# PN-CourseWork/02689-AdvancedNumericalAlgorithmP3

Hardware: AMD Instinct MI355X
Metric: steady-state time-steps/sec at N=256 Re=1000 (higher is better)
Workload: dtype f64; 1 GPU; solver=spectral (SG) N=256 Re=1000 fp64, full solve() iteration (dt, 4 RK stages + BCs, change/residual norms, E/Z/P), fluid from rest; N=256, trials_per_gpu=1, parallelism=1 independent trial(s), one per GPU

## Files before the change

02689-advancednumericalalgorithmp3_amd/csrc/ldc_kernels.hip:

```cpp

#include <hip/hip_runtime.h>
#include <stdint.h>
#include <stdlib.h>
#include <string.h>
#include <mutex>
#include <new>
#include <type_traits>
#include <vector>

#include "ldc_hip.h"
#include "ldc_fv_common.inc"

namespace {

#ifdef LDC_TIMING
#define LDC_ABL(x, bits) ((x).ablate & (bits))
#else
#define LDC_ABL(x, bits) 0
#endif

constexpr int kWaves = 4;
constexpr int kThreads = 256;
constexpr int kMfmaBounds = 512;

__device__ __forceinline__ v4d ldfrag(const double* X, int ld, int r0, int k0, int lane) {
  return *reinterpret_cast<const v4d*>(X + (size_t)(r0 + (lane & 15)) * ld + k0 + 4 * (lane >> 4));
}

#define LDC_GLOBAL __attribute__((address_space(1)))
__device__ __forceinline__ v4d ldpk(const double* XK, int NB, int R, int G, int lane) {
  return *(const LDC_GLOBAL v4d*)(XK + (((size_t)(R * NB + G) << 6) + lane) * 4);
}
template <typename T>
__device__ __forceinline__ T gl(const T* p, size_t i) {
  return ((const LDC_GLOBAL T*)p)[i];
}

__device__ __forceinline__ __amdgpu_buffer_rsrc_t raw_rsrc(const double* base) {
  return __builtin_amdgcn_make_buffer_rsrc((void*)base, 0, -1, 0x00020000);
}
typedef unsigned int v4u __attribute__((ext_vector_type(4)));
typedef double v2d_t __attribute__((ext_vector_type(2)));
template <bool COH>
__device__ __forceinline__ v4d ldpk_t(const double* XK, int NB, int R, int G, int lane) {
  if constexpr (!COH) {
    return ldpk(XK, NB, R, G, lane);
  } else {
    const __amdgpu_buffer_rsrc_t r = raw_rsrc(XK);
    const int off = ((((R * NB + G) << 6) + lane) * 4) * (int)sizeof(double);
    const v2d_t lo = __builtin_bit_cast(v2d_t, __builtin_amdgcn_raw_buffer_load_b128(r, off, 0, 16));
    const v2d_t hi = __builtin_bit_cast(v2d_t, __builtin_amdgcn_raw_buffer_load_b128(r, off + 16, 0, 16));
    return (v4d){lo[0], lo[1], hi[0], hi[1]};
  }
}
template <bool COH, typename T>
__device__ __forceinline__ T gl_t(const T* p, size_t i) {
  if constexpr (!COH) return gl(p, i);
  else return __hip_atomic_load((const LDC_GLOBAL T*)p + i, __ATOMIC_RELAXED, __HIP_MEMORY_SCOPE_AGENT);
}

__device__ __forceinline__ void st_out2(double* p, double v0, double v1, int wt) {
  const v2d_t v = {v0, v1};
  if (wt) asm volatile("global_store_dwordx4 %0, %1, off sc1\n\ts_nop 1" :: "v"((LDC_GLOBAL v2d_t*)p), "v"(v) : "memory");
  else *(LDC_GLOBAL v2d_t*)p = v;
}
__device__ __forceinline__ void st_out(double* p, double v, int wt) {
  if (wt) __hip_atomic_store((LDC_GLOBAL double*)p, v, __ATOMIC_RELAXED, __HIP_MEMORY_SCOPE_AGENT);
  else *(LDC_GLOBAL double*)p = v;
}

template <typename T>
__device__ __forceinline__ T sload(const T* p) {
  return *(const __attribute__((address_space(4))) T*)p;
}

template <int CTRL>
__device__ __forceinline__ double dpp_move(double x) {
  const long long b = __builtin_bit_cast(long long, x);
  const int lo = __builtin_amdgcn_update_dpp(0, (int)b, CTRL, 0xf, 0xf, true);
  const int hi = __builtin_amdgcn_update_dpp(0, (int)(b >> 32), CTRL, 0xf, 0xf, true);
  return __builtin_bit_cast(double, ((long long)hi << 32) | (unsigned int)lo);
}
__device__ __forceinline__ double lane_value(double x, int l) {
  const long long b = __builtin_bit_cast(long long, x);
  const int lo = __builtin_amdgcn_readlane((int)b, l), hi = __builtin_amdgcn_readlane((int)(b >> 32), l);
  return __builtin_bit_cast(double, ((long long)hi << 32) | (unsigned int)lo);
// ... 2521 lines not shown
```

02689-advancednumericalalgorithmp3_amd/csrc/ldc_wide_kernel.inc:

```

constexpr int kWT = 16;
constexpr int kWTmin = 6;
constexpr int kWD2 = 6;
constexpr int kWD = 4;

struct WArgs {
  int M, LD, NB, T;
  int tail;
  int Mx, My;
  int with_diag;
  double nu, beta2;
  const double *DxK, *D2xK, *DyK, *D2yK, *GxFK, *GyFK;
  const double *ulid, *wx, *wy;
  double *U, *UT, *V, *VT, *P;
  double *UK[3], *UTK[3], *VK[3], *VTK[3], *PK[3];
  double *PTK[3];
  double *WK, *WTK;
  const double *IxF, *IyF;
  const double *Dx, *D2x, *Dy, *D2y, *GxF, *GyF;
  const double *DxL, *D2xL, *DyL, *D2yL;
  double* wedge;
  double* jobs;
  double* ring;
  double* rvec;
  double *part4, *partZ0, *partP0;
  long long stride;
  FinalArgs fin;
  unsigned* flags;
  unsigned* giveup;
  double* stamps;
};
constexpr int kWStampPoints = 12;
constexpr int kWStampsPerWg = kStageWaves * 4 * kWStampPoints;

struct WLaunch {
  int B, n_iters;
  const WArgs* trials;
  WArgs one;
};
static_assert(sizeof(WLaunch) <= 4096, "WLaunch must fit the kernel-argument segment");
typedef const __attribute__((address_space(4))) WArgs WArgsC;

struct WLds {
  int OPS, RES, AXY, RNG, EYX, RY, TOT, RSUM, TOTAL;
};
__host__ __device__ inline WLds wlds_of(int T) {
  WLds l;
  l.OPS = 0;
  l.RES = l.OPS + 4 * T * 256;
// ... 55 lines not shown
  }
}
__device__ __forceinline__ void wgive_up(WArgsC& a, TrialState* S) {
  S->abort = 1;
  __hip_atomic_store((LDC_GLOBAL unsigned*)a.giveup, 1u, __ATOMIC_RELAXED, __HIP_MEMORY_SCOPE_AGENT);
}

__device__ __forceinline__ bool wbar(WArgsC& a, unsigned& phaseA, int T, int bx, int I, int J, int tid, TrialState* S, bool all,
                                     double* stp = nullptr) {
  asm volatile("s_waitcnt vmcnt(0)" ::: "memory");
  WSTAMP(7);
  __syncthreads();
  WSTAMP(8);
  ++phaseA;
  if (tid < 64) {
    if (tid == 0) __hip_atomic_store((LDC_GLOBAL unsigned*)a.flags + 32 * bx, phaseA, __ATOMIC_RELAXED, __HIP_MEMORY_SCOPE_AGENT);
    if (!wwait_flags(a.flags, phaseA, T, I, J, all, tid) && tid == 0) wgive_up(a, S);
    WSTAMP(9);
  }
  __syncthreads();
  WSTAMP(10);
  return S->abort == 0;
}

__device__ __forceinline__ v4d wld4(const double* base, size_t i) {
  const __amdgpu_buffer_rsrc_t r = raw_rsrc(base);
  const int off = (int)(i * sizeof(double));
  const v2d_t lo = __builtin_bit_cast(v2d_t, __builtin_amdgcn_raw_buffer_load_b128(r, off, 0, 16));
  const v2d_t hi = __builtin_bit_cast(v2d_t, __builtin_amdgcn_raw_buffer_load_b128(r, off + 16, 0, 16));
  return (v4d){lo[0], lo[1], hi[0], hi[1]};
}
__device__ __forceinline__ int wrows_padded(int nwg) { return (nwg + 3) & ~3; }

template <bool CONST_A>
__device__ __forceinline__ void wchain2(v4d& r0, v4d& r1, const double* p0, const double* p1, const double* pan, int NB,
                                        int prow, int T, int lane) {
  constexpr int D = kWD2;
  v4d f[D];
#pragma unroll
  for (int d = 0; d < D; ++d) {
    f[d] = ldpk_t<true>(pan, NB, prow, d, lane);
    __builtin_amdgcn_sched_barrier(0);
  }
  v4d c0[2], c1[2];
#pragma unroll
  for (int h = 0; h < 2; ++h) { c0[h] = (v4d){0.0, 0.0, 0.0, 0.0}; c1[h] = (v4d){0.0, 0.0, 0.0, 0.0}; }
  auto mm = [&](const v4d& x, int g) {
    const v4d k0 = wfrag_lds(p0 + g * 256, lane), k1 = wfrag_lds(p1 + g * 256, lane);
#pragma unroll
    for (int s = 0; s < 4; ++s) {
      if (CONST_A) { c0[s & 1] = MFMA_F64(k0[s], x[s], c0[s & 1]); c1[s & 1] = MFMA_F64(k1[s], x[s], c1[s & 1]); }
      else         { c0[s & 1] = MFMA_F64(x[s], k0[s], c0[s & 1]); c1[s & 1] = MFMA_F64(x[s], k1[s], c1[s & 1]); }
    }
  };
  int g = 0;
  for (; g + 2 * D <= T; g += D) {
#pragma unroll
    for (int d = 0; d < D; ++d) {
      mm(f[d], g + d);
      f[d] = ldpk_t<true>(pan, NB, prow, g + d + D, lane);
      __builtin_amdgcn_sched_barrier(0);
    }
  }
  const int rest = T - g - D;
#pragma unroll
  for (int d = 0; d < D; ++d) {
    mm(f[d], g + d);
    if (d < rest) f[d] = ldpk_t<true>(pan, NB, prow, g + d + D, lane);
  }
#pragma unroll
  for (int d = 0; d < D; ++d)
    if (d < rest) mm(f[d], g + D + d);
  r0 = xadd(c0[0], c0[1]);
  r1 = xadd(c1[0], c1[1]);
}

template <bool OP_LDS, bool CONST_A>
__device__ __forceinline__ v4d wchain1(const double* opl, const double* opk, int oprow, const double* pan, int prow, int NB,
                                       int ng, int lane, int g0 = 0) {
  constexpr int D = kWD;
  v4d f[D], o[D];
#pragma unroll
  for (int d = 0; d < D; ++d) {
    f[d] = ldpk_t<true>(pan, NB, prow, g0 + (d < ng ? d : ng - 1), lane);
    if (!OP_LDS) o[d] = ldpk(opk, NB, oprow, g0 + (d < ng ? d : ng - 1), lane);
    __builtin_amdgcn_sched_barrier(0);
  }
  v4d c[4];
#pragma unroll
  for (int s = 0; s < 4; ++s) c[s] = (v4d){0.0, 0.0, 0.0, 0.0};
  auto mm = [&](const v4d& x, const v4d& k) {
#pragma unroll
    for (int s = 0; s < 4; ++s) c[s] = CONST_A ? MFMA_F64(k[s], x[s], c[s]) : MFMA_F64(x[s], k[s], c[s]);
  };
  int g = 0;
  for (; g + 2 * D <= ng; g += D) {
#pragma unroll
    for (int d = 0; d < D; ++d) {
      mm(f[d], OP_LDS ? wfrag_lds(opl + (g0 + g + d) * 256, lane) : o[d]);
      f[d] = ldpk_t<true>(pan, NB, prow, g0 + g + d + D, lane);
      if (!OP_LDS) o[d] = ldpk(opk, NB, oprow, g0 + g + d + D, lane);
      __builtin_amdgcn_sched_barrier(0);
    }
  }
  const int rest = ng - g - D;
#pragma unroll
  for (int d = 0; d < D; ++d) {
    if (g + d < ng) mm(f[d], OP_LDS ? wfrag_lds(opl + (g0 + g + d) * 256, lane) : o[d]);
    if (d < rest) {
      f[d] = ldpk_t<true>(pan, NB, prow, g0 + g + d + D, lane);
      if (!OP_LDS) o[d] = ldpk(opk, NB, oprow, g0 + g + d + D, lane);
    }
  }
#pragma unroll
  for (int d = 0; d < D; ++d)
    if (d < rest) mm(f[d], OP_LDS ? wfrag_lds(opl + (g0 + g + D + d) * 256, lane) : o[d]);
  return xadd(xadd(c[0], c[1]), xadd(c[2], c[3]));
}

__device__ __forceinline__ void wput(double* lds, const WLds& Ld, int slot, const v4d& acc, int lane) {
#pragma unroll
  for (int r = 0; r < 4; ++r) lds[Ld.RES + (slot * 4 + r) * 64 + lane] = acc[r];
}

__device__ __forceinline__ double wave_total(double x) { return quad_sum(row16_sum(x)); }
__device__ __forceinline__ double wave_top(double x) { return quad_max(row16_max(x)); }


__device__ __forceinline__ void wring_partials(WArgsC& a, const WLds& Ld, const XNode& n, double* lds, double pn, int bx,
                                               int lane, int wv) {
  double* dst = a.ring + (size_t)wopaque_s(bx) * 64;
  const double eyc[2] = {lds[Ld.EYX + n.tj], lds[Ld.EYX + 16 + n.tj]};
  const double exc[2] = {lds[Ld.EYX + 32 + n.ti], lds[Ld.EYX + 48 + n.ti]};
#pragma unroll
  for (int c = 0; c < 2; ++c) {
    const double r = row16_sum(pn * eyc[c]);
    if ((lane & 15) == 0) wst1(dst + c * 16 + n.ti, r);
    const double q = quad_sum(exc[c] * pn);
    if (lane < 16) lds[Ld.RY + (wv * 2 + c) * 16 + lane] = q;
  }
}
__device__ __forceinline__ void wring_partials_finish(WArgsC& a, const WLds& Ld, const double* lds, int bx, int tid) {
  if (tid < 32) {
    const double* r = lds + Ld.RY + tid;
// ... 12 lines not shown
  double s = 0.0;
#pragma unroll
  for (int L = 0; L < kWT; ++L) s += (L < T) ? t[L] : 0.0;
  wst1(a.rvec + (size_t)v * 16 * T + 16 * B + r, s);
}
__device__ __forceinline__ void wvec_line(const double* vec, size_t off, const double* opK, int oprow, int NB, int T, int lane_,
                                          double* out, const double* opl = nullptr) {
  const int lane = wopaque(lane_);
  double s = 0.0;
#pragma unroll
  for (int g0 = 0; g0 < kWT; g0 += 8) {
    if (g0 < T) {
      v4d G[8], A[8];
#pragma unroll
      for (int g = 0; g < 8; ++g) {
        const int gc = g0 + g < T ? g0 + g : T - 1;
        if (opl == nullptr) G[g] = ldpk(opK, NB, oprow, gc, lane);
        A[g] = wld4(vec, off + 16 * gc + 4 * (lane >> 4));
      }
#pragma unroll
      for (int g = 0; g < 8; ++g) {
        if (g0 + g < T) {
          const v4d Gg = (opl == nullptr) ? G[g] : wfrag_lds(opl + (g0 + g) * 256, lane);
          s = nm_madd(Gg[0], A[g][0], s); s = nm_madd(Gg[1], A[g][1], s);
          s = nm_madd(Gg[2], A[g][2], s); s = nm_madd(Gg[3], A[g][3], s);
        }
      }
    }
  }
  s = quad_sum(s);
  if (lane < 16) out[lane] = s;
}
struct WVecHalf { double a[8]; };
__device__ __forceinline__ void wvec_issue(WVecHalf& h, const double* vec, size_t off, int g0, int ng, int lane_) {
  const int lane = wopaque(lane_);
#pragma unroll
  for (int g = 0; g < 8; ++g) h.a[g] = xld(vec, off + 16 * (g0 + (g < ng ? g : ng - 1)) + 4 * (lane >> 4) + (lane & 3));
}
__device__ __forceinline__ void wvec_finish(const WVecHalf& h, const double* opl, const double* opK, int oprow, int NB, int g0, int ng,
                                            int lane_, double* out) {
  const int lane = wopaque(lane_);
  v4d G[8];
  if (opl == nullptr) {
#pragma unroll
    for (int g = 0; g < 8; ++g) G[g] = ldpk(opK, NB, oprow, g0 + (g < ng ? g : ng - 1), lane);
  }
  double s0 = 0.0, s1 = 0.0, s2 = 0.0, s3 = 0.0;
#pragma unroll
  for (int g = 0; g < 8; ++g) {
    if (g < ng) {
      const v4d Gg = (opl == nullptr) ? G[g] : wfrag_lds(opl + (g0 + g) * 256, lane);
      s0 = nm_madd(Gg[0], dpp_move<0x00>(h.a[g]), s0); s1 = nm_madd(Gg[1], dpp_move<0x55>(h.a[g]), s1);
      s2 = nm_madd(Gg[2], dpp_move<0xAA>(h.a[g]), s2); s3 = nm_madd(Gg[3], dpp_move<0xFF>(h.a[g]), s3);
    }
  }
  const double s = quad_sum((s0 + s1) + (s2 + s3));
  if (lane < 16) out[lane] = s;
}
__device__ __forceinline__ void wring_line(WArgsC& a, int T, int blk, int lane, int kind, int c, double* out) {
  wvec_line(a.rvec, (size_t)(2 * kind + c) * 16 * T, kind == 0 ? a.GxFK : a.GyFK, blk, a.NB, T, lane, out);
}
__device__ __forceinline__ double wvv(const double* row, const double* vec, size_t off, int n, int lane_) {
  const int lane = wopaque(lane_);
  double s = 0.0;
  if (4 * lane < n) {
    const v4d r = *(const LDC_GLOBAL v4d*)(row + 4 * lane);
    const v4d x = wld4(vec, off + 4 * lane);
    s = nm_madd(r[0], x[0], s); s = nm_madd(r[1], x[1], s); s = nm_madd(r[2], x[2], s); s = nm_madd(r[3], x[3], s);
  }
  return wave_total(s);
// ... 28 lines not shown
  jb.cd[2] = xld(base, WJ_CD2 * 16 + r); jb.cd[3] = xld(base, WJ_CD3 * 16 + r);
  jb.ce[0] = xld(base, WJ_CE0 * 16 + r); jb.ce[1] = xld(base, WJ_CE1 * 16 + r);
  jb.ce[2] = xld(base, WJ_CE2 * 16 + r); jb.ce[3] = xld(base, WJ_CE3 * 16 + r);
  jb.pgs = xld(base, WJ_PGS * 16 + r); jb.pgr = xld(base, WJ_PGR * 16 + r);
  jb.omega = xld(base, WJ_OMEGA * 16 + r); jb.wq = xld(base, WJ_WQ * 16 + r); jb.opl = xld(base, WJ_OPL * 16 + r);
  jb.am1 = xld(base, WJ_UNI * 16 + 0); jb.am2 = xld(base, WJ_UNI * 16 + 1); jb.wc = xld(base, WJ_UNI * 16 + 2);
}
__device__ __forceinline__ void wjob_store(WArgsC& a, const WJob& jb, int T, int lane_, bool all) {
  const int lane = wopaque(lane_);
  double* base = a.jobs + (size_t)wjob_id(jb.kind, jb.blk, T) * kWJobDoubles;
  if (lane < 16) {
    wst1(base + WJ_PGS * 16 + lane, jb.pgs); wst1(base + WJ_PGR * 16 + lane, jb.pgr); wst1(base + WJ_OMEGA * 16 + lane, jb.omega);
    if (all) {
      wst1(base + WJ_UE * 16 + lane, jb.ue); wst1(base + WJ_VE * 16 + lane, jb.ve);
      wst1(base + WJ_CD0 * 16 + lane, jb.cd[0]); wst1(base + WJ_CD1 * 16 + lane, jb.cd[1]);
      wst1(base + WJ_CD2 * 16 + lane, jb.cd[2]); wst1(base + WJ_CD3 * 16 + lane, jb.cd[3]);
      wst1(base + WJ_CE0 * 16 + lane, jb.ce[0]); wst1(base + WJ_CE1 * 16 + lane, jb.ce[1]);
      wst1(base + WJ_CE2 * 16 + lane, jb.ce[2]); wst1(base + WJ_CE3 * 16 + lane, jb.ce[3]);
      wst1(base + WJ_WQ * 16 + lane, jb.wq); wst1(base + WJ_OPL * 16 + lane, jb.opl);
      if (lane == 0) { wst1(base + WJ_UNI * 16 + 0, jb.am1); wst1(base + WJ_UNI * 16 + 1, jb.am2); wst1(base + WJ_UNI * 16 + 2, jb.wc); }
    }
  }
}
enum { WR_JOBLINE = 64, WR_EXTRA = 96, WR_CGX = 97, WR_CGY = 98, WR_CPX = 99, WR_CPY = 100, WR_JOBRING2 = 104 };

struct WEdgeLoads { double ra[4], rb[4]; v4d f0[4], f1[4]; };
template <int MODE, bool DIAGV>
__device__ __forceinline__ void wedge_issue(WEdgeLoads& w, WArgsC& a, int kind, int blk, const XStageIo io, int T, int w4, int lane_) {
  const int lane = wopaque(lane_);
  const int NB = a.NB;
  const size_t rowm = (size_t)(a.M - 1) * a.LD;
  const double *pan0, *pan1, *rA, *rB;
  if (MODE == 1) {
    pan0 = kind == 0 ? a.VTK[io.in] : a.UK[io.in]; pan1 = kind == 0 ? a.PTK[io.pin] : a.PK[io.pin];
    rA = (kind == 0 ? a.Dx : a.Dy) + rowm; rB = (kind == 0 ? a.GxF : a.GyF) + rowm;
  } else if (MODE == 3) {
    pan0 = kind == 0 ? a.WTK : a.WK; pan1 = pan0;
    rA = (kind == 0 ? a.Dx : a.Dy) + rowm; rB = rA;
  } else {
    pan0 = kind == 0 ? a.UTK[io.in] : a.UK[io.in]; pan1 = kind == 0 ? a.VTK[io.in] : a.VK[io.in];
    rA = (kind == 0 ? a.Dx : a.Dy) + rowm; rB = (kind == 0 ? a.D2x : a.D2y) + rowm;
  }
  constexpr bool use0 = !(MODE == 1 && !DIAGV), use1 = MODE != 3;
#pragma unroll
  for (int m = 0; m < 4; ++m) {
    const int g = w4 + 4 * m, gc = g < T ? g : T - 1;
    const int ko = 16 * gc + 4 * (lane >> 4) + (lane & 3);
    w.ra[m] = *(const LDC_GLOBAL double*)(rA + ko);
    w.rb[m] = use1 ? *(const LDC_GLOBAL double*)(rB + ko) : w.ra[m];
    if (g >= T) { w.ra[m] = 0.0; w.rb[m] = 0.0; }
  }
#pragma unroll
  for (int m = 0; m < 4; ++m) {
    const int g = w4 + 4 * m, gc = g < T ? g : T - 1;
    w.f0[m] = use0 ? ldpk_t<true>(pan0, NB, blk, gc, lane) : (v4d){0.0, 0.0, 0.0, 0.0};
    w.f1[m] = use1 ? ldpk_t<true>(pan1, NB, blk, gc, lane) : w.f0[m];
  }
}
template <int MODE, bool DIAGV>
__device__ __forceinline__ void wedge_dots(const WEdgeLoads& w, const WLds& Ld, double* lds, int w4, int lane_) {
  const int lane = wopaque(lane_);
  constexpr bool use0 = !(MODE == 1 && !DIAGV), use1 = MODE != 3;
  double acc[4] = {0.0, 0.0, 0.0, 0.0};
#pragma unroll
  for (int m = 0; m < 4; ++m) {
    const v4d va = {dpp_move<0x00>(w.ra[m]), dpp_move<0x55>(w.ra[m]), dpp_move<0xAA>(w.ra[m]), dpp_move<0xFF>(w.ra[m])};
    v4d vb = va;
    if (use1) vb = (v4d){dpp_move<0x00>(w.rb[m]), dpp_move<0x55>(w.rb[m]), dpp_move<0xAA>(w.rb[m]), dpp_move<0xFF>(w.rb[m])};
    if (MODE == 1) { if (use0) fma4(acc[0], w.f0[m], va); fma4(acc[1], w.f1[m], vb); }
    if (MODE == 3) fma4(acc[0], w.f0[m], va);
    if (MODE == 4) {
#pragma unroll
      for (int e = 0; e < 4; ++e) {
        acc[0] = fma(w.f0[m][e], va[e], acc[0]); acc[1] = fma(w.f0[m][e], vb[e], acc[1]);
        acc[2] = fma(w.f1[m][e], va[e], acc[2]); acc[3] = fma(w.f1[m][e], vb[e], acc[3]);
      }
    }
  }
#pragma unroll
  for (int d = 0; d < 4; ++d) {
    if ((MODE == 1 && d < 2) || (MODE == 3 && d < 1) || MODE == 4) {
      const double x = quad_sum(acc[d]);
      if (lane < 16) lds[Ld.AXY + (w4 * 5 + (MODE == 3 ? 4 : d)) * 16 + lane] = x;
    }
  }
}
template <int MODE, bool DIAGV>
__device__ __forceinline__ void wedge_stream(WArgsC& a, const WLds& Ld, double* lds, int kind, int blk, const XStageIo io,
                                             int T, int w4, int lane) {
// ... 244 lines not shown
  constexpr bool PUBZ = DIAGV && K == 2;
  constexpr double alphas[4] = {0.25, 1.0 / 3.0, 0.5, 1.0};
  constexpr int bin[4] = {0, 1, 2, 1}, bout[4] = {1, 2, 1, 0};
  const XStageIo io = {bin[K], bout[K], bin[K], bout[K], alphas[K], K};
  const int T = wopaque_s(T_), bx = wopaque_s(bx_), I = wopaque_s(I_), J = wopaque_s(J_);
  WJob jb;
  jb.kind = TAIL ? jkind : -1; jb.blk = jblk;
  jb.ue = jb.ve = jb.am1 = jb.am2 = jb.pgs = jb.pgr = jb.omega = jb.wq = jb.opl = jb.wc = 0.0;
#pragma unroll
  for (int d = 0; d < 4; ++d) { jb.cd[d] = 0.0; jb.ce[d] = 0.0; }
  const int tid = wopaque((int)threadIdx.x), lane = tid & 63;
  const int wv = __builtin_amdgcn_readfirstlane(tid >> 6);
#ifdef LDC_TIMING
  double* const stp = stamp ? a.stamps + (size_t)bx * kWStampsPerWg + (wv * 4 + K) * kWStampPoints : nullptr;
#else
  double* const stp = nullptr; (void)stamp;
#endif
  WSTAMP(0);
  const int NB = a.NB, nwg = T * T;
  constexpr bool has_p = SP || LAST;
  const double* ops = lds + Ld.OPS;
  const int iLast = (a.Mx - 1) / 16, jLast = (a.My - 1) / 16;
  double* rsum = lds + Ld.RSUM;
  double* rng = lds + Ld.RNG;
  const bool job = TAIL && jb.kind >= 0;
  v4d fx[PS_N + 2];
  WFoldState fs = {false, false, 0.0, 0.0};
  WEdgeLoads jw;
  WVecHalf jvh;
  double wre = 0.0, wce = 0.0;
  if (wv < 4) {
    if (TAIL && DIAGE == 2) { wre = xld(a.wedge, (size_t)n.j); wce = xld(a.wedge, (size_t)16 * kWT + n.i); }
    const bool xrole = wv < 2;
    const double* pan = wv == 0 ? a.UTK[io.in] : wv == 1 ? a.VTK[io.in] : wv == 2 ? a.UK[io.in] : a.VK[io.in];
    const double* p0 = ops + (xrole ? 0 : 2) * T * 256;
    v4d c0, c1;
    if (xrole) wchain2<true>(c0, c1, p0, p0 + T * 256, pan, NB, J, T, lane);
    else wchain2<false>(c0, c1, p0, p0 + T * 256, pan, NB, I, T, lane);
    WSTAMP(1);
    wput(lds, Ld, wv == 0 ? XR_UX : wv == 1 ? XR_VX : wv == 2 ? XR_UY : XR_VY, c0, lane);
    wput(lds, Ld, wv == 0 ? XR_UXX : wv == 1 ? XR_VXX : wv == 2 ? XR_UYY : XR_VYY, c1, lane);
  } else {
    if (PUBZ && wv == 7 && lane == 0) {
      const double* r = rsum;
      const double x = (((r[0] + r[1]) + (r[2] + r[3])) + ((r[4] + r[5]) + (r[6] + r[7]))) +
                       (((r[8] + r[9]) + (r[10] + r[11])) + ((r[12] + r[13]) + (r[14] + r[15])));
      const int step0 = S->step;
      wst1(a.partZ0 + (size_t)((step0 > 0 ? step0 - 1 : 0) & 1) * a.stride + wopaque_s(bx), TAIL ? x + r[16] : x);
    }
    if (GPV) {
      constexpr bool THREE = !(SP && K == 3);
      const int c1 = THREE ? (2 * T + 1) / 3 : T;
      if (wv == 4) wput(lds, Ld, XR_PX, wchain1<false, true>(nullptr, a.GxFK, I, a.PTK[io.pin], J, NB, c1, lane), lane);
      else if (wv == 5) wput(lds, Ld, XR_PY, wchain1<false, false>(nullptr, a.GyFK, J, a.PK[io.pin], I, NB, c1, lane), lane);
      else if (THREE && wv == 6) {
        wput(lds, Ld, XR_WX, wchain1<false, true>(nullptr, a.GxFK, I, a.PTK[io.pin], J, NB, T - c1, lane, c1), lane);
        wput(lds, Ld, XR_WY, wchain1<false, false>(nullptr, a.GyFK, J, a.PK[io.pin], I, NB, T - c1, lane, c1), lane);
      }
    }
    if (AGRADW) {
      const int h0 = (T + 1) / 2, g0 = wv < 6 ? 0 : h0, ng = wv < 6 ? h0 : T - h0;
      if ((wv & 1) == 0) wput(lds, Ld, wv == 4 ? XR_PX : XR_WX, wchain1<true, true>(ops, nullptr, 0, a.WTK, J, NB, ng, lane, g0), lane);
      else wput(lds, Ld, wv == 5 ? XR_PY : XR_WY, wchain1<true, false>(ops + 2 * T * 256, nullptr, 0, a.WK, I, NB, ng, lane, g0), lane);
    }
    if (RRED && wv == 7 && I == J) wring_reduce(a, T, I, lane);
    if (K == 0 && wv == 7 && fold) {
      fs = wfold_dt(a, S, T, I, J, lane, phaseA, fx, stp);
      wfold_step(a, S, fs, lane);
    }
    if (TAIL && LAST && job) {
      const size_t rowm = (size_t)(a.M - 1) * a.LD;
      const int q0 = (wv - 4) * T / 4, q1 = (wv - 3) * T / 4;
      if (DIAGV && jb.kind < 2) wvec_issue(jvh, a.wedge, jb.kind == 0 ? 0 : (size_t)16 * kWT, q0, q1 - q0, lane);
      if (wv >= 6) wjob_load(a, jb, T, lane);
      if (jb.kind < 2) wedge_issue<4, DIAGV>(jw, a, jb.kind, jb.blk, io, T, wv - 4, lane);
      if (DIAGV && jb.kind == 2 && wv == 7) {
        const double* jbase = a.jobs + (size_t)wjob_id(2, 0, T) * kWJobDoubles;
        const int l4 = 4 * wopaque(lane), n4 = 16 * T;
        jw.ra[0] = xld(jbase, WJ_UNI * 16 + 0); jw.ra[1] = xld(jbase, WJ_UNI * 16 + 1); jw.ra[2] = xld(jbase, WJ_UNI * 16 + 2);
        const bool in = l4 < n4;
        const int lc = in ? l4 : 0;
        jw.f0[0] = *(const LDC_GLOBAL v4d*)(a.Dx + rowm + lc); jw.f0[1] = wld4(a.wedge, (size_t)16 * kWT + lc);
        jw.f0[2] = *(const LDC_GLOBAL v4d*)(a.Dy + rowm + lc); jw.f0[3] = wld4(a.wedge, (size_t)lc);
        if (!in) { jw.f0[0] = (v4d){0.0, 0.0, 0.0, 0.0}; jw.f0[2] = jw.f0[0]; }
      }
      WSTAMP(1);
    }
    if (TAIL && K == 1 && wv == 6 && job) wjob_load(a, jb, T, lane);
    if (RING3 && wv >= 6) {
      if (!wwait_flags(a.flags, phaseA, T, I, J, true, lane)) {
        if (lane == 0) wgive_up(a, S);
      } else {
        if (J == 0 || J == jLast) wring(a, Ld, lds, T, I, J, lane, wv - 6, 0, J == 0 ? 0 : 1);
        if (I == 0 || I == iLast) wring(a, Ld, lds, T, I, J, lane, wv - 6, 1, I == 0 ? 0 : 1);
      }
    }
  }
  WSTAMP(2);
  __syncthreads();
  WSTAMP(3);
  if (S->abort != 0) return false;
  double v[PS_N], ev[PS_N];
#pragma unroll
  for (int q = 0; q < PS_N; ++q) ev[q] = 0.0;
  if (TAIL && K == 1 && wv == 6 && job) { wedge_finish<1, DIAGV>(a, Ld, lds, jb, lane, ev); wjob_store(a, jb, T, lane, false); }
  if (TAIL && LAST && job && wv >= 4) {
    if (jb.kind < 2) wedge_dots<4, DIAGV>(jw, Ld, lds, wv - 4, lane);
    if (DIAGV && jb.kind < 2) {
      const int q0 = (wv - 4) * T / 4, q1 = (wv - 3) * T / 4;
      wvec_finish(jvh, jb.kind == 0 ? ops + 2 * T * 256 : ops, nullptr, 0, NB, q0, q1 - q0, lane, lds + Ld.AXY + 320 + 16 * (wv - 4));
    }
    if (DIAGV && jb.kind == 2 && wv == 7) {
      double sx = 0.0, sy = 0.0;
#pragma unroll
      for (int e = 0; e < 4; ++e) { sx = nm_madd(jw.f0[0][e], jw.f0[1][e], sx); sy = nm_madd(jw.f0[2][e], jw.f0[3][e], sy); }
      const double gxc = wave_total(sx) + jw.ra[0] * jw.ra[2], gyc = wave_total(sy) + jw.ra[1] * jw.ra[2];
      if (lane == 0) { rng[WR_CGX] = gxc; rng[WR_CGY] = gyc; }
    }
  }
  if (tid < 256) {
    auto C = [&](int slot) { return lds[Ld.RES + (slot * 4 + wv) * 64 + lane]; };
    double ux = C(XR_UX), vx = C(XR_VX), uy = C(XR_UY), vy = C(XR_VY);
    double lu = C(XR_UXX) + C(XR_UYY), lv = C(XR_VXX) + C(XR_VYY);
    if (TAIL) { ux += tn.cux; vx += tn.cvx; uy += tn.cuy; vy += tn.cvy; lu += tn.clu; lv += tn.clv; }
    const int blkIJ = I * NB + J, blkJI = J * NB + I;
    double dsum = 0.0;
    if (GPV) {
      constexpr bool THREE = !(SP && K == 3);
      n.px = n.valid ? (THREE ? C(XR_PX) + C(XR_WX) : C(XR_PX)) : 0.0;
      n.py = n.valid ? (THREE ? C(XR_PY) + C(XR_WY) : C(XR_PY)) : 0.0;
    }
    if (RINGE) {
      if (n.rc >= 0) n.px = rng[n.ti];
      if (n.rr >= 0) n.py = rng[32 + n.tj];
    }
    if (RING3) {
      if (n.rc >= 0) n.px = rng[n.ti] + rng[16 + n.ti];
      if (n.rr >= 0) n.py = rng[32 + n.tj] + rng[48 + n.tj];
    }
    if (DIAGE == 1) {
      const double w = n.valid ? (vx - uy) : 0.0;
      wst(a.WK, blkIJ, n.oU, w);
      wst(a.WTK, blkJI, n.oT, w);
      dsum = n.valid ? n.wq * w * w : 0.0;
    }
    if (DIAGE == 2) {
      double gx = C(XR_PX) + C(XR_WX), gy = C(XR_PY) + C(XR_WY);
      if (TAIL) { gx = nm_madd(tn.dxl, wre, gx); gy = nm_madd(wce, tn.dyl, gy); }
      dsum = n.valid ? n.wq * nm_sq2(gx, gy) : 0.0;
    }
    const double Ru = nm_momentum(n.uc, n.vc, ux, uy, n.px, a.nu, lu);
    const double Rv = nm_momentum(n.uc, n.vc, vx, vy, n.py, a.nu, lv);
    const double Rp = nm_continuity(a.beta2, ux, vy);
    const double adt = io.alpha * S->dt;
    double un = nm_madd(adt, Ru, n.u0), vn = nm_madd(adt, Rv, n.v0);
    if (!n.valid) { un = 0.0; vn = 0.0; }
    else if (n.lid) { un = n.lidv; vn = 0.0; }
    else if (n.wall) { un = 0.0; vn = 0.0; }
    wst(a.UK[io.out], blkIJ, n.oU, un);
    wst(a.UTK[io.out], blkJI, n.oT, un);
    wst(a.VK[io.out], blkIJ, n.oU, vn);
    wst(a.VTK[io.out], blkJI, n.oT, vn);
    double pn = 0.0;
    if (has_p) {
      pn = n.interior ? nm_madd(adt, Rp, n.p0) : 0.0;
      wst(a.PK[io.pout], blkIJ, n.oU, pn);
      wst(a.PTK[io.pout], blkJI, n.oT, pn);
      if (RPROD) wring_partials(a, Ld, n, lds, pn, bx, lane, wv);
    }
    if (LAST) {
      const double du = un - n.u0, dv = vn - n.v0;
      v[PS_DU2] = n.valid ? du * du : 0.0;
      v[PS_DV2] = n.valid ? dv * dv : 0.0;
      v[PS_U02] = n.valid ? n.u0 * n.u0 : 0.0;
      v[PS_V02] = n.valid ? n.v0 * n.v0 : 0.0;
      v[PS_RU2] = n.valid ? Ru * Ru : 0.0;
      v[PS_RV2] = n.valid ? Rv * Rv : 0.0;
      v[PS_RP2] = n.interior ? Rp * Rp : 0.0;
      v[PS_E] = n.valid ? n.wq * nm_sq2(un, vn) : 0.0;
      v[PS_UMAX] = fabs(un);
      v[PS_VMAX] = fabs(vn);
      n.u0 = un; n.v0 = vn; n.p0 = pn;
    }
    if (DIAGE != 0) {
      const double r = row16_sum(dsum);
      if ((lane & 15) == 0) rsum[n.ti] = r;
    }
    n.uc = un; n.vc = vn;
  }
  WSTAMP(4);
  if (LAST || RPROD) {
    __syncthreads();
    WSTAMP(5);
    if (RPROD) wring_partials_finish(a, Ld, lds, bx, tid);
    if (LAST) {
      constexpr int RS = TAIL ? 272 : 256;
      double* red = lds + Ld.RES;
      if (tid < 256) {
#pragma unroll
// ... 80 lines not shown
  }
  __syncthreads();
  WSTAMP(10);
  return S->abort == 0;
}

template <bool SP, bool DIAGV, bool TAIL>
__global__ __launch_bounds__(kStageThreads, 2) void wide_kernel(const WLaunch L) {
  static_assert(!(SP && DIAGV), "the smoother carries no diagnostics");
  static_assert(!(SP && TAIL), "the tail layout is built for SG");
  extern __shared__ __attribute__((aligned(16))) double lds[];
  __shared__ TrialState S;
  const int tid = threadIdx.x, lane = tid & 63;
  const int wv = __builtin_amdgcn_readfirstlane(tid >> 6);
  WArgsC& a0 = L.trials ? *(WArgsC*)(uintptr_t)L.trials
                        : *(WArgsC*)((kernarg_ptr)__builtin_amdgcn_kernarg_segment_ptr() + __builtin_offsetof(WLaunch, one));
  const int T = a0.T, nwg = T * T;
  const int trial = (int)blockIdx.x / nwg, bx = (int)blockIdx.x % nwg;
  WArgsC& a = L.trials ? *(WArgsC*)(uintptr_t)(L.trials + trial) : a0;
  const WLds Ld = wlds_of(T);
  const int NB = a.NB, M = a.M, LD = a.LD;
  const int I = bx / T, J = bx % T;
  if (a.fin.ctrl[LDC_CTRL_DONE] != 0) return;
  if (tid == 0) {
    S.done = a.fin.ctrl[LDC_CTRL_DONE]; S.iter = a.fin.ctrl[LDC_CTRL_ITER]; S.step = a.fin.ctrl[LDC_CTRL_STEP];
    S.flushed = a.fin.ctrl[LDC_CTRL_FLUSHED]; S.pdone = a.fin.ctrl[LDC_CTRL_PDONE]; S.drows = a.fin.ctrl[LDC_CTRL_DROWS];
    S.dt = a.fin.scal[LDC_SCAL_DT]; S.umax = a.fin.scal[LDC_SCAL_UMAX]; S.vmax = a.fin.scal[LDC_SCAL_VMAX];
    S.abort = 0; S.arrive = 0u; S.dtp = 0.0;
  }
  for (int q = tid; q < 4 * T * 256; q += kStageThreads) {
    const int p = q / (T * 256), r = q - p * (T * 256), g = r >> 8, e = r & 255;
    const double* src = p == 0 ? a.DxK : p == 1 ? a.D2xK : p == 2 ? a.DyK : a.D2yK;
    const int row = p < 2 ? I : J;
    lds[Ld.OPS + (p * T + g) * 256 + ((e & 3) >> 1) * 128 + (e >> 2) * 2 + (e & 1)] = src[((size_t)(row * NB + g) << 8) + e];
  }
  XNode n;
  n.ti = 4 * (wv & 3) + (lane >> 4); n.tj = lane & 15;
  n.i = 16 * I + n.ti; n.j = 16 * J + n.tj;
  n.oU = xpk(n.ti, n.tj); n.oT = xpk(n.tj, n.ti);
  const int Mx = a.Mx, My = a.My;
  n.valid = (n.i < Mx) && (n.j < My);
  n.interior = (n.i >= 1) && (n.i <= Mx - 2) && (n.j >= 1) && (n.j <= My - 2);
  n.lid = n.valid && (n.j == My - 1);
  n.wall = n.valid && (n.i == 0 || n.i == Mx - 1 || n.j == 0);
  n.rc = !n.valid ? -1 : n.j == 0 ? 0 : n.j == My - 1 ? 1 : -1;
  n.rr = !n.valid ? -1 : n.i == 0 ? 0 : n.i == Mx - 1 ? 1 : -1;
  n.u0 = n.v0 = n.p0 = n.px = n.py = n.lidv = n.wq = 0.0;
  const size_t ij = (size_t)n.i * LD + n.j;
  if (tid < 64) {
    const int c = (tid >> 4) & 1, e = tid & 15;
    const size_t row = c ? (size_t)((tid < 32 ? My : Mx) - 1) * LD : 0;
    lds[Ld.EYX + tid] = (tid < 32) ? a.IyF[row + 16 * J + e] : a.IxF[row + 16 * I + e];
  }
  if (tid < 256) {
    n.u0 = a.U[ij]; n.v0 = a.V[ij]; n.p0 = a.P[ij];
    n.lidv = a.ulid[n.i];
    n.wq = a.wx[n.i] * a.wy[n.j];
    wst(a.UK[0], I * NB + J, n.oU, n.u0); wst(a.UTK[0], J * NB + I, n.oT, n.u0);
    wst(a.VK[0], I * NB + J, n.oU, n.v0); wst(a.VTK[0], J * NB + I, n.oT, n.v0);
    wst(a.PK[0], I * NB + J, n.oU, n.p0);
    wst(a.PTK[0], J * NB + I, n.oT, n.p0);
  }
  if (!SP) {
    __syncthreads();
    if (tid < 256) wring_partials(a, Ld, n, lds, n.p0, bx, lane, wv);
    __syncthreads();
    wring_partials_finish(a, Ld, lds, bx, tid);
  }
  n.uc = n.u0; n.vc = n.v0;
  WTailNode tn = {0.0, 0.0, 0.0, 0.0, 0.0, 0.0, 0.0, 0.0};
  int jkind = -1, jblk = 0;
  if (TAIL) {
    if (tid < 256) {
      const size_t rowm = (size_t)(M - 1) * LD;
      const double dxl = a.DxL[n.i], d2xl = a.D2xL[n.i], dyl = a.DyL[n.j], d2yl = a.D2yL[n.j];
      const double ue = a.U[rowm + n.j], ve = a.V[rowm + n.j];
      const double un = a.UT[rowm + n.i], vn = a.VT[rowm + n.i];
      tn.cux = dxl * ue; tn.cvx = dxl * ve; tn.cuy = un * dyl; tn.cvy = vn * dyl;
      tn.clu = nm_madd(d2xl, ue, un * d2yl); tn.clv = nm_madd(d2xl, ve, vn * d2yl);
      tn.dxl = dxl; tn.dyl = dyl;
    }
    jkind = (I == J) ? 0 : (J == (I + 1) % T) ? 1 : (I == 1 && J == 3) ? 2 : -1;
    jblk = jkind == 0 ? J : I;
    if (wv == 6 && jkind >= 0) {
      double* jbase = a.jobs + (size_t)wjob_id(jkind, jblk, T) * kWJobDoubles;
      if (xld(jbase, WJ_UNI * 16 + 3) != kWJobTag) {
        WJob jb;
        wjob_init(a, jb, T, I, J, lane);
        wjob_store(a, jb, T, lane, true);
        if (lane == 0) wst1(jbase + WJ_UNI * 16 + 3, kWJobTag);
      }
    }
    if (tid < 16) lds[Ld.RSUM + 16 + tid] = 0.0;
// ... 4 lines not shown
  for (int it = 0; alive && it < L.n_iters; ++it) {
    if (S.done != 0) break;
#ifdef LDC_TIMING
    const bool stamp = a.stamps != nullptr && it == L.n_iters - 1;
#else
    const bool stamp = false;
#endif
    alive = wstage<SP, DIAGV, TAIL, 0>(a, Ld, n, tn, jkind, jblk, lds, &S, phaseA, T, bx, I, J, pending, stamp);
    if (!alive) break;
    pending = false;
    if (S.done != 0) break;
    alive = wstage<SP, DIAGV, TAIL, 1>(a, Ld, n, tn, jkind, jblk, lds, &S, phaseA, T, bx, I, J, false, stamp);
    if (!alive) break;
    alive = wstage<SP, DIAGV, TAIL, 2>(a, Ld, n, tn, jkind, jblk, lds, &S, phaseA, T, bx, I, J, false, stamp);
    if (!alive) break;
    alive = wstage<SP, DIAGV, TAIL, 3>(a, Ld, n, tn, jkind, jblk, lds, &S, phaseA, T, bx, I, J, false, stamp);
    pending = true;
  }
  if (!alive) return;
  if (pending) {
    if (wv == 7) {
      v4d fx[PS_N + 2];
      const WFoldState fs = wfold_dt(a, &S, T, I, J, lane, phaseA, fx, nullptr);
      wfold_step(a, &S, fs, lane);
      wfold_record(a, Ld, lds, &S, T, lane, bx == 0, fs, fx, nullptr);
    }
    __syncthreads();
    if (S.abort != 0) return;
  }
  double* tu = lds + Ld.RES;
  double* tv = tu + 16 * 17;
  if (tid < 256) {
    a.U[ij] = n.u0; a.V[ij] = n.v0; a.P[ij] = n.p0;
    tu[n.ti * 17 + n.tj] = n.u0; tv[n.ti * 17 + n.tj] = n.v0;
  }
  __syncthreads();
  if (tid < 256) {
    const int tr = tid >> 4, tc = tid & 15;
    const size_t ot = (size_t)(16 * J + tr) * LD + 16 * I + tc;
    a.UT[ot] = tu[tc * 17 + tr];
    a.VT[ot] = tv[tc * 17 + tr];
  }
  if (bx == 0 && tid == 0) {
    a.fin.ctrl[LDC_CTRL_DONE] = S.done; a.fin.ctrl[LDC_CTRL_ITER] = S.iter; a.fin.ctrl[LDC_CTRL_STEP] = S.step;
    a.fin.ctrl[LDC_CTRL_FLUSHED] = S.flushed; a.fin.ctrl[LDC_CTRL_PDONE] = S.pdone; a.fin.ctrl[LDC_CTRL_DROWS] = S.drows;
    a.fin.ctrl[LDC_CTRL_LIVE] = 0;
    a.fin.scal[LDC_SCAL_DT] = S.dt; a.fin.scal[LDC_SCAL_UMAX] = S.umax; a.fin.scal[LDC_SCAL_VMAX] = S.vmax;
  }
}
```

Before: 28210 steps/s.

## Drop duplicate row-major packed panels; read y-role operands from transposed panels

Each stage used to write every packed field (U, V, P, W) in two layouts, row-major and transposed. Now only the transposed layout is stored. The y-direction consumers read it through new strided loaders (ldpk_rows, ldpk_k4s), and the LDS operator staging and the edge vectors are reindexed to the swapped k ordering. This removes half of the per-stage packed-panel global stores. The cost is narrower, less coalesced 64-bit loads on the y-role paths, and only the initial UK/VK/PK copies are written at kernel exit.

```diff
diff --git a/02689-advancednumericalalgorithmp3_amd/csrc/ldc_kernels.hip b/02689-advancednumericalalgorithmp3_amd/csrc/ldc_kernels.hip
--- a/02689-advancednumericalalgorithmp3_amd/csrc/ldc_kernels.hip
+++ b/02689-advancednumericalalgorithmp3_amd/csrc/ldc_kernels.hip
@@ -52,6 +52,19 @@
     const v2d_t hi = __builtin_bit_cast(v2d_t, __builtin_amdgcn_raw_buffer_load_b128(r, off + 16, 0, 16));
     return (v4d){lo[0], lo[1], hi[0], hi[1]};
   }
+}
+__device__ __forceinline__ v4d ldpk_rows(const double* XK, int NB, int G, int R, int lane) {
+  const __amdgpu_buffer_rsrc_t r = raw_rsrc(XK);
+  const int j = lane & 15, q = lane >> 4;
+  const int off = (((G * NB + R) << 8) + ((j >> 2) << 6) + 4 * q + (j & 3)) * (int)sizeof(double);
+  v4d x;
+#pragma unroll
+  for (int s = 0; s < 4; ++s) x[s] = __builtin_bit_cast(double, __builtin_amdgcn_raw_buffer_load_b64(r, off + 128 * s, 0, 16));
+  return x;
+}
+__device__ __forceinline__ v4d ldpk_k4s(const double* XK, int NB, int R, int G, int lane) {
+  const LDC_GLOBAL double* p = (const LDC_GLOBAL double*)XK + ((size_t)(R * NB + G) << 8) + 4 * (lane & 15) + (lane >> 4);
+  return (v4d){p[0], p[64], p[128], p[192]};
 }
 template <bool COH, typename T>
 __device__ __forceinline__ T gl_t(const T* p, size_t i) {
diff --git a/02689-advancednumericalalgorithmp3_amd/csrc/ldc_wide_kernel.inc b/02689-advancednumericalalgorithmp3_amd/csrc/ldc_wide_kernel.inc
--- a/02689-advancednumericalalgorithmp3_amd/csrc/ldc_wide_kernel.inc
+++ b/02689-advancednumericalalgorithmp3_amd/csrc/ldc_wide_kernel.inc
@@ -13,8 +13,9 @@
   const double *DxK, *D2xK, *DyK, *D2yK, *GxFK, *GyFK;
   const double *ulid, *wx, *wy;
   double *U, *UT, *V, *VT, *P;
-  double *UK[3], *UTK[3], *VK[3], *VTK[3], *PK[3];
+  double *UTK[3], *VTK[3];
   double *PTK[3];
+  double *UK[3], *VK[3], *PK[3];
   double *WK, *WTK;
   const double *IxF, *IyF;
   const double *Dx, *D2x, *Dy, *D2y, *GxF, *GyF;
@@ -136,6 +137,17 @@
 }
 __device__ __forceinline__ int wrows_padded(int nwg) { return (nwg + 3) & ~3; }
 
+template <bool YROLE>
+__device__ __forceinline__ v4d wldst(const double* pan, int NB, int prow, int g, int lane) {
+  if constexpr (YROLE) return ldpk_rows(pan, NB, g, prow, lane);
+  else return ldpk_t<true>(pan, NB, prow, g, lane);
+}
+template <bool YROLE>
+__device__ __forceinline__ v4d wldop(const double* opk, int NB, int oprow, int g, int lane) {
+  if constexpr (YROLE) return ldpk_k4s(opk, NB, oprow, g, lane);
+  else return ldpk(opk, NB, oprow, g, lane);
+}
+
 template <bool CONST_A>
 __device__ __forceinline__ void wchain2(v4d& r0, v4d& r1, const double* p0, const double* p1, const double* pan, int NB,
                                         int prow, int T, int lane) {
@@ -143,7 +155,7 @@
   v4d f[D];
 #pragma unroll
   for (int d = 0; d < D; ++d) {
-    f[d] = ldpk_t<true>(pan, NB, prow, d, lane);
+    f[d] = wldst<!CONST_A>(pan, NB, prow, d, lane);
     __builtin_amdgcn_sched_barrier(0);
   }
   v4d c0[2], c1[2];
@@ -162,7 +174,7 @@
 #pragma unroll
     for (int d = 0; d < D; ++d) {
       mm(f[d], g + d);
-      f[d] = ldpk_t<true>(pan, NB, prow, g + d + D, lane);
+      f[d] = wldst<!CONST_A>(pan, NB, prow, g + d + D, lane);
       __builtin_amdgcn_sched_barrier(0);
     }
   }
@@ -170,7 +182,7 @@
 #pragma unroll
   for (int d = 0; d < D; ++d) {
     mm(f[d], g + d);
-    if (d < rest) f[d] = ldpk_t<true>(pan, NB, prow, g + d + D, lane);
+    if (d < rest) f[d] = wldst<!CONST_A>(pan, NB, prow, g + d + D, lane);
   }
 #pragma unroll
   for (int d = 0; d < D; ++d)
@@ -186,8 +198,8 @@
   v4d f[D], o[D];
 #pragma unroll
   for (int d = 0; d < D; ++d) {
-    f[d] = ldpk_t<true>(pan, NB, prow, g0 + (d < ng ? d : ng - 1), lane);
-    if (!OP_LDS) o[d] = ldpk(opk, NB, oprow, g0 + (d < ng ? d : ng - 1), lane);
+    f[d] = wldst<!CONST_A>(pan, NB, prow, g0 + (d < ng ? d : ng - 1), lane);
+    if (!OP_LDS) o[d] = wldop<!CONST_A>(opk, NB, oprow, g0 + (d < ng ? d : ng - 1), lane);
     __builtin_amdgcn_sched_barrier(0);
   }
   v4d c[4];
@@ -202,8 +214,8 @@
 #pragma unroll
     for (int d = 0; d < D; ++d) {
       mm(f[d], OP_LDS ? wfrag_lds(opl + (g0 + g + d) * 256, lane) : o[d]);
-      f[d] = ldpk_t<true>(pan, NB, prow, g0 + g + d + D, lane);
-      if (!OP_LDS) o[d] = ldpk(opk, NB, oprow, g0 + g + d + D, lane);
+      f[d] = wldst<!CONST_A>(pan, NB, prow, g0 + g + d + D, lane);
+      if (!OP_LDS) o[d] = wldop<!CONST_A>(opk, NB, oprow, g0 + g + d + D, lane);
       __builtin_amdgcn_sched_barrier(0);
     }
   }
@@ -212,8 +224,8 @@
   for (int d = 0; d < D; ++d) {
     if (g + d < ng) mm(f[d], OP_LDS ? wfrag_lds(opl + (g0 + g + d) * 256, lane) : o[d]);
     if (d < rest) {
-      f[d] = ldpk_t<true>(pan, NB, prow, g0 + g + d + D, lane);
-      if (!OP_LDS) o[d] = ldpk(opk, NB, oprow, g0 + g + d + D, lane);
+      f[d] = wldst<!CONST_A>(pan, NB, prow, g0 + g + d + D, lane);
+      if (!OP_LDS) o[d] = wldop<!CONST_A>(opk, NB, oprow, g0 + g + d + D, lane);
     }
   }
 #pragma unroll
@@ -292,10 +304,11 @@
   if (lane < 16) out[lane] = s;
 }
 struct WVecHalf { double a[8]; };
-__device__ __forceinline__ void wvec_issue(WVecHalf& h, const double* vec, size_t off, int g0, int ng, int lane_) {
+__device__ __forceinline__ void wvec_issue(WVecHalf& h, const double* vec, size_t off, int g0, int ng, int lane_, bool k4s = false) {
   const int lane = wopaque(lane_);
-#pragma unroll
-  for (int g = 0; g < 8; ++g) h.a[g] = xld(vec, off + 16 * (g0 + (g < ng ? g : ng - 1)) + 4 * (lane >> 4) + (lane & 3));
+  const int e = k4s ? 4 * (lane & 3) + (lane >> 4) : 4 * (lane >> 4) + (lane & 3);
+#pragma unroll
+  for (int g = 0; g < 8; ++g) h.a[g] = xld(vec, off + 16 * (g0 + (g < ng ? g : ng - 1)) + e);
 }
 __device__ __forceinline__ void wvec_finish(const WVecHalf& h, const double* opl, const double* opK, int oprow, int NB, int g0, int ng,
                                             int lane_, double* out) {
@@ -390,29 +403,38 @@
   const size_t rowm = (size_t)(a.M - 1) * a.LD;
   const double *pan0, *pan1, *rA, *rB;
   if (MODE == 1) {
-    pan0 = kind == 0 ? a.VTK[io.in] : a.UK[io.in]; pan1 = kind == 0 ? a.PTK[io.pin] : a.PK[io.pin];
+    pan0 = kind == 0 ? a.VTK[io.in] : a.UTK[io.in]; pan1 = a.PTK[io.pin];
     rA = (kind == 0 ? a.Dx : a.Dy) + rowm; rB = (kind == 0 ? a.GxF : a.GyF) + rowm;
   } else if (MODE == 3) {
-    pan0 = kind == 0 ? a.WTK : a.WK; pan1 = pan0;
+    pan0 = a.WTK; pan1 = pan0;
     rA = (kind == 0 ? a.Dx : a.Dy) + rowm; rB = rA;
   } else {
-    pan0 = kind == 0 ? a.UTK[io.in] : a.UK[io.in]; pan1 = kind == 0 ? a.VTK[io.in] : a.VK[io.in];
+    pan0 = a.UTK[io.in]; pan1 = a.VTK[io.in];
     rA = (kind == 0 ? a.Dx : a.Dy) + rowm; rB = (kind == 0 ? a.D2x : a.D2y) + rowm;
   }
   constexpr bool use0 = !(MODE == 1 && !DIAGV), use1 = MODE != 3;
 #pragma unroll
   for (int m = 0; m < 4; ++m) {
     const int g = w4 + 4 * m, gc = g < T ? g : T - 1;
-    const int ko = 16 * gc + 4 * (lane >> 4) + (lane & 3);
+    const int ko = 16 * gc + (kind == 1 ? 4 * (lane & 3) + (lane >> 4) : 4 * (lane >> 4) + (lane & 3));
     w.ra[m] = *(const LDC_GLOBAL double*)(rA + ko);
     w.rb[m] = use1 ? *(const LDC_GLOBAL double*)(rB + ko) : w.ra[m];
     if (g >= T) { w.ra[m] = 0.0; w.rb[m] = 0.0; }
   }
-#pragma unroll
-  for (int m = 0; m < 4; ++m) {
-    const int g = w4 + 4 * m, gc = g < T ? g : T - 1;
-    w.f0[m] = use0 ? ldpk_t<true>(pan0, NB, blk, gc, lane) : (v4d){0.0, 0.0, 0.0, 0.0};
-    w.f1[m] = use1 ? ldpk_t<true>(pan1, NB, blk, gc, lane) : w.f0[m];
+  if (kind == 1) {
+#pragma unroll
+    for (int m = 0; m < 4; ++m) {
+      const int g = w4 + 4 * m, gc = g < T ? g : T - 1;
+      w.f0[m] = use0 ? ldpk_rows(pan0, NB, gc, blk, lane) : (v4d){0.0, 0.0, 0.0, 0.0};
+      w.f1[m] = use1 ? ldpk_rows(pan1, NB, gc, blk, lane) : w.f0[m];
+    }
+  } else {
+#pragma unroll
+    for (int m = 0; m < 4; ++m) {
+      const int g = w4 + 4 * m, gc = g < T ? g : T - 1;
+      w.f0[m] = use0 ? ldpk_t<true>(pan0, NB, blk, gc, lane) : (v4d){0.0, 0.0, 0.0, 0.0};
+      w.f1[m] = use1 ? ldpk_t<true>(pan1, NB, blk, gc, lane) : w.f0[m];
+    }
   }
 }
 template <int MODE, bool DIAGV>
@@ -723,7 +745,7 @@
   if (wv < 4) {
     if (TAIL && DIAGE == 2) { wre = xld(a.wedge, (size_t)n.j); wce = xld(a.wedge, (size_t)16 * kWT + n.i); }
     const bool xrole = wv < 2;
-    const double* pan = wv == 0 ? a.UTK[io.in] : wv == 1 ? a.VTK[io.in] : wv == 2 ? a.UK[io.in] : a.VK[io.in];
+    const double* pan = (wv & 1) == 0 ? a.UTK[io.in] : a.VTK[io.in];
     const double* p0 = ops + (xrole ? 0 : 2) * T * 256;
     v4d c0, c1;
     if (xrole) wchain2<true>(c0, c1, p0, p0 + T * 256, pan, NB, J, T, lane);
@@ -743,16 +765,16 @@
       constexpr bool THREE = !(SP && K == 3);
       const int c1 = THREE ? (2 * T + 1) / 3 : T;
       if (wv == 4) wput(lds, Ld, XR_PX, wchain1<false, true>(nullptr, a.GxFK, I, a.PTK[io.pin], J, NB, c1, lane), lane);
-      else if (wv == 5) wput(lds, Ld, XR_PY, wchain1<false, false>(nullptr, a.GyFK, J, a.PK[io.pin], I, NB, c1, lane), lane);
+      else if (wv == 5) wput(lds, Ld, XR_PY, wchain1<false, false>(nullptr, a.GyFK, J, a.PTK[io.pin], I, NB, c1, lane), lane);
       else if (THREE && wv == 6) {
         wput(lds, Ld, XR_WX, wchain1<false, true>(nullptr, a.GxFK, I, a.PTK[io.pin], J, NB, T - c1, lane, c1), lane);
-        wput(lds, Ld, XR_WY, wchain1<false, false>(nullptr, a.GyFK, J, a.PK[io.pin], I, NB, T - c1, lane, c1), lane);
+        wput(lds, Ld, XR_WY, wchain1<false, false>(nullptr, a.GyFK, J, a.PTK[io.pin], I, NB, T - c1, lane, c1), lane);
       }
     }
     if (AGRADW) {
       const int h0 = (T + 1) / 2, g0 = wv < 6 ? 0 : h0, ng = wv < 6 ? h0 : T - h0;
       if ((wv & 1) == 0) wput(lds, Ld, wv == 4 ? XR_PX : XR_WX, wchain1<true, true>(ops, nullptr, 0, a.WTK, J, NB, ng, lane, g0), lane);
-      else wput(lds, Ld, wv == 5 ? XR_PY : XR_WY, wchain1<true, false>(ops + 2 * T * 256, nullptr, 0, a.WK, I, NB, ng, lane, g0), lane);
+      else wput(lds, Ld, wv == 5 ? XR_PY : XR_WY, wchain1<true, false>(ops + 2 * T * 256, nullptr, 0, a.WTK, I, NB, ng, lane, g0), lane);
     }
     if (RRED && wv == 7 && I == J) wring_reduce(a, T, I, lane);
     if (K == 0 && wv == 7 && fold) {
@@ -762,7 +784,7 @@
     if (TAIL && LAST && job) {
       const size_t rowm = (size_t)(a.M - 1) * a.LD;
       const int q0 = (wv - 4) * T / 4, q1 = (wv - 3) * T / 4;
-      if (DIAGV && jb.kind < 2) wvec_issue(jvh, a.wedge, jb.kind == 0 ? 0 : (size_t)16 * kWT, q0, q1 - q0, lane);
+      if (DIAGV && jb.kind < 2) wvec_issue(jvh, a.wedge, jb.kind == 0 ? 0 : (size_t)16 * kWT, q0, q1 - q0, lane, jb.kind == 0);
       if (wv >= 6) wjob_load(a, jb, T, lane);
       if (jb.kind < 2) wedge_issue<4, DIAGV>(jw, a, jb.kind, jb.blk, io, T, wv - 4, lane);
       if (DIAGV && jb.kind == 2 && wv == 7) {
@@ -814,7 +836,7 @@
     double ux = C(XR_UX), vx = C(XR_VX), uy = C(XR_UY), vy = C(XR_VY);
     double lu = C(XR_UXX) + C(XR_UYY), lv = C(XR_VXX) + C(XR_VYY);
     if (TAIL) { ux += tn.cux; vx += tn.cvx; uy += tn.cuy; vy += tn.cvy; lu += tn.clu; lv += tn.clv; }
-    const int blkIJ = I * NB + J, blkJI = J * NB + I;
+    const int blkJI = J * NB + I;
     double dsum = 0.0;
     if (GPV) {
       constexpr bool THREE = !(SP && K == 3);
@@ -831,7 +853,6 @@
     }
     if (DIAGE == 1) {
       const double w = n.valid ? (vx - uy) : 0.0;
-      wst(a.WK, blkIJ, n.oU, w);
       wst(a.WTK, blkJI, n.oT, w);
       dsum = n.valid ? n.wq * w * w : 0.0;
     }
@@ -848,14 +869,11 @@
     if (!n.valid) { un = 0.0; vn = 0.0; }
     else if (n.lid) { un = n.lidv; vn = 0.0; }
     else if (n.wall) { un = 0.0; vn = 0.0; }
-    wst(a.UK[io.out], blkIJ, n.oU, un);
     wst(a.UTK[io.out], blkJI, n.oT, un);
-    wst(a.VK[io.out], blkIJ, n.oU, vn);
     wst(a.VTK[io.out], blkJI, n.oT, vn);
     double pn = 0.0;
     if (has_p) {
       pn = n.interior ? nm_madd(adt, Rp, n.p0) : 0.0;
-      wst(a.PK[io.pout], blkIJ, n.oU, pn);
       wst(a.PTK[io.pout], blkJI, n.oT, pn);
       if (RPROD) wring_partials(a, Ld, n, lds, pn, bx, lane, wv);
     }
@@ -1002,12 +1020,13 @@
     const int p = q / (T * 256), r = q - p * (T * 256), g = r >> 8, e = r & 255;
     const double* src = p == 0 ? a.DxK : p == 1 ? a.D2xK : p == 2 ? a.DyK : a.D2yK;
     const int row = p < 2 ? I : J;
-    lds[Ld.OPS + (p * T + g) * 256 + ((e & 3) >> 1) * 128 + (e >> 2) * 2 + (e & 1)] = src[((size_t)(row * NB + g) << 8) + e];
+    const int ln = p >= 2 ? 16 * (e & 3) + ((e >> 2) & 15) : e >> 2, sk = p >= 2 ? e >> 6 : e & 3;
+    lds[Ld.OPS + (p * T + g) * 256 + (sk >> 1) * 128 + ln * 2 + (sk & 1)] = src[((size_t)(row * NB + g) << 8) + e];
   }
   XNode n;
   n.ti = 4 * (wv & 3) + (lane >> 4); n.tj = lane & 15;
   n.i = 16 * I + n.ti; n.j = 16 * J + n.tj;
-  n.oU = xpk(n.ti, n.tj); n.oT = xpk(n.tj, n.ti);
+  n.oU = 0; n.oT = xpk(n.tj, n.ti);
   const int Mx = a.Mx, My = a.My;
   n.valid = (n.i < Mx) && (n.j < My);
   n.interior = (n.i >= 1) && (n.i <= Mx - 2) && (n.j >= 1) && (n.j <= My - 2);
@@ -1026,9 +1045,8 @@
     n.u0 = a.U[ij]; n.v0 = a.V[ij]; n.p0 = a.P[ij];
     n.lidv = a.ulid[n.i];
     n.wq = a.wx[n.i] * a.wy[n.j];
-    wst(a.UK[0], I * NB + J, n.oU, n.u0); wst(a.UTK[0], J * NB + I, n.oT, n.u0);
-    wst(a.VK[0], I * NB + J, n.oU, n.v0); wst(a.VTK[0], J * NB + I, n.oT, n.v0);
-    wst(a.PK[0], I * NB + J, n.oU, n.p0);
+    wst(a.UTK[0], J * NB + I, n.oT, n.u0);
+    wst(a.VTK[0], J * NB + I, n.oT, n.v0);
     wst(a.PTK[0], J * NB + I, n.oT, n.p0);
   }
   if (!SP) {
@@ -1099,6 +1117,8 @@
   double* tv = tu + 16 * 17;
   if (tid < 256) {
     a.U[ij] = n.u0; a.V[ij] = n.v0; a.P[ij] = n.p0;
+    const size_t ku = ((size_t)(I * NB + J) << 8) + xpk(n.ti, n.tj);
+    a.UK[0][ku] = n.u0; a.VK[0][ku] = n.v0; a.PK[0][ku] = n.p0;
     tu[n.ti * 17 + n.tj] = n.u0; tv[n.ti * 17 + n.tj] = n.v0;
   }
   __syncthreads();
```

After: 28210 steps/s, median of 3. Within noise of the previous version (-0.0%).
